# dymensionxyz/cometbft

Measured on AMD Instinct MI355X. Metric: Ed25519 verifs/sec at 1/2/4/8 GPUs + p50 VerifyCommit latency, 150 vals, higher is better.
Workload: dtype u32

## Files before the change

### cometbft_amd/_native.py

```python
from __future__ import annotations

import ctypes
import os

_HERE = os.path.dirname(os.path.abspath(__file__))
LIB_PATH = os.environ.get("CMTV_LIBRARY") or os.path.join(_HERE, "libcmtverify.so")

CMTV_OK = 0
CMTV_EINVAL = -1
CMTV_ENODEV = -2
CMTV_ENOMEM = -3
CMTV_EHIP = -4
CMTV_ERCCL = -5
CMTV_ECOMMIT = -6

MODE_GO_STDLIB = 0
MODE_ZIP215 = 1

VERIFY_COMMIT = 0
VERIFY_COMMIT_LIGHT = 1
VERIFY_COMMIT_LIGHT_TRUSTING = 2

KEY_ED25519 = 0
KEY_SECP256K1 = 1
# ... 39 lines not shown
                ("flags", ctypes.c_uint32), ("reserved", ctypes.c_uint32)]


class cmtv_stats(ctypes.Structure):
    _fields_ = [("calls", ctypes.c_uint64), ("signatures", ctypes.c_uint64), ("invalid", ctypes.c_uint64),
                ("kernel_launches", ctypes.c_uint64), ("device_ms", ctypes.c_double),
                ("last_kernel_ms", ctypes.c_double), ("cache_hits", ctypes.c_uint64),
                ("cache_entries", ctypes.c_uint64), ("keyed_launches", ctypes.c_uint64),
                ("sharded_calls", ctypes.c_uint64), ("gathers", ctypes.c_uint64),
                ("faults_injected", ctypes.c_uint64), ("n_devices", ctypes.c_uint32), ("rccl", ctypes.c_uint32),
                ("fused_sign_bytes", ctypes.c_uint64), ("device_failures", ctypes.c_uint64),
                ("reshards", ctypes.c_uint64), ("late_k_waves", ctypes.c_uint64),
                ("live_devices", ctypes.c_uint32), ("secp_batch_launches", ctypes.c_uint32),
                ("timed_calls", ctypes.c_uint64), ("rccl_failures", ctypes.c_uint64),
                ("polled_calls", ctypes.c_uint64), ("direct_chunks", ctypes.c_uint64),
                ("masked_chunks", ctypes.c_uint64), ("isolated_calls", ctypes.c_uint64)]


class cmtv_device_stats(ctypes.Structure):
    _fields_ = [("ordinal", ctypes.c_int32), ("failed", ctypes.c_uint32), ("calls", ctypes.c_uint64),
                ("signatures", ctypes.c_uint64), ("kernel_launches", ctypes.c_uint64),
                ("device_ms", ctypes.c_double), ("timed_calls", ctypes.c_uint64)]


_u8p = ctypes.POINTER(ctypes.c_uint8)


class cmtv_block_id(ctypes.Structure):
    _fields_ = [("hash", _u8p), ("hash_len", ctypes.c_uint32), ("psh_total", ctypes.c_uint32),
                ("psh_hash", _u8p), ("psh_hash_len", ctypes.c_uint32)]

# ... 151 lines not shown
```

### cometbft_amd/csrc/hs_helper.h

```cpp
#pragma once
#include "devtables.h"
#include "quad.h"

namespace cmtv {

constexpr int kHsCombPre = 6, kHsCombPreFused = 3, kHsCombPreSr = 0;
constexpr uint32_t kHsSlotU2 = 3 * 5 * 64;
constexpr uint32_t kHsTabU2 = 2 * 9 * 5 * 64;

__device__ __forceinline__ int hs_comb_pre(uint32_t hs_tune, int dflt) {
  const int c = (hs_tune & 0xFFu) ? (int)(hs_tune & 0xFFu) - 1 : dflt;
  return c > 16 ? 16 : c;
}

__device__ __forceinline__ int hs_workgroup_windows(uint32_t flags, uint32_t t) {
  const bool wide = __ballot(t < 48 && (flags & 2u) != 0) != 0;
  int W = HS_WINDOWS;
#pragma unroll 1
  for (int x = HS_WINDOWS; x < HS_MAX_WINDOWS; x++) W += __ballot(t < 48 && (int)((flags >> 8) & 0xFFu) > x) ? 1 : 0;
  return wide ? HS_WIDE_WINDOWS : W;
}

template <class Clock>
__device__ __forceinline__ void hs_helper_windows(const SigPrep& p, int W, const BComb16& bc, const uint2* tabs,
                                                  uint2* ring, uint32_t t, const Clock& clock, uint64_t& hwait) {
  const uint32_t slot = t < 48 ? t : 47;
  const bool r_flip = (p.flags & 1u) != 0;
  uint32_t tA[8], tR[8];
  hs_digits16(tA, p.k1, W);
  hs_digits16(tR, p.k2, W);
  sc_shift_out(tA, 4);
  sc_shift_out(tR, 4);
  const uint2* tw = tabs + (slot >> 4) * kHsTabU2;
  const uint32_t qb = 4 * (slot & 15);
  auto rd = [&](int P, int e, int c, fe& r) {
    const uint2* src = tw + (P * 9 + e) * 5 * 64 + qb + c;
#pragma unroll
    for (int k = 0; k < 5; k++) {
      const uint2 x = src[k * 64];
      r.v[2 * k] = x.x;
      r.v[2 * k + 1] = x.y;
    }
  };
  auto put = [&](uint2* dst, const fe* out) {
    if (t < 48) {
#pragma unroll
      for (int c = 0; c < 4; c++)
#pragma unroll
        for (int k = 0; k < 5; k++)
          dst[(slot >> 4) * 320 + k * 64 + qb + c] = make_uint2(out[c].v[2 * k], out[c].v[2 * k + 1]);
    }
  };
#pragma unroll 1
  for (int win = W - 2; win >= 0; win--) {
    const int dA = (int)sc_shift_out(tA, 4) - 8;
    const int dR = (int)sc_shift_out(tR, 4) - 8;
    fe out[4];
    h_window_addend(out, rd, dA, dR, r_flip);
    put(ring + (win & 1) * kHsSlotU2, out);
    const uint64_t c0 = clock();
    __syncthreads();
    hwait += clock() - c0;
  }
  fe out[4], d2;
  fe_sub(out[0], bc.P.Y, bc.P.X);
  fe_add(out[1], bc.P.Y, bc.P.X);
  fe_add(out[2], bc.P.Z, bc.P.Z);
  fe_const_d2(d2);
  fe_mul(out[3], bc.P.T, d2);
  put(ring + kHsSlotU2, out);
}

__device__ __forceinline__ void hs_slot_load(const uint2* sl, uint32_t wave, uint32_t t, fe& c) {
#pragma unroll
  for (int k = 0; k < 5; k++) {
    const uint2 x = sl[wave * 320 + k * 64 + t];
    c.v[2 * k] = x.x;
    c.v[2 * k + 1] = x.y;
  }
}

}
```

### cometbft_amd/csrc/kernels.h

```cpp
#pragma once
#include <hip/hip_runtime.h>
#include <stdint.h>

namespace cmtv {

constexpr uint32_t kBtabWords = (3 * 128 + 3 * 32768 + 16 * 32768) * 36;
constexpr uint32_t kAtabWordsPerLane = 320;
constexpr uint32_t kCombWords = 32 * 128 * 32;
constexpr uint32_t kCombScratchWordsPerKey = 128 * 320;

constexpr uint32_t kFormLane = 0, kFormQuad = 1, kFormOct2 = 2, kFormRow = 3, kFormRow4 = 4;
constexpr uint32_t kFormMask = 0xFF, kLaunchForceWide = 0x100;
constexpr uint32_t kKeyedRow = 0, kKeyedQuad = 1, kKeyedLane = 2;

constexpr uint32_t kRowSlots = 256, kRowSlotWords = 1024, kRowMaxCap = 4 * (kRowSlotWords - 16);
struct RowSlot {
  uint32_t* words = nullptr;
  uint64_t* tagged = nullptr;
  uint32_t seq = 0;
};

struct SbFuse {
  const void* tmpls = nullptr;
  const uint8_t* blob = nullptr;
  const uint32_t* tidx = nullptr;
  const uint8_t* flag = nullptr;
  const int64_t* sec = nullptr;
  const int32_t* nanos = nullptr;
};
constexpr uint32_t kSbFuseMaxMsg = 192;

constexpr uint32_t kDiagLateK = 0, kDiagWords = 4;
constexpr uint32_t kKeyedWaitDefault = 1u << 22;

hipError_t launch_btab_init(uint32_t* d_rows, hipStream_t s);
hipError_t launch_verify(uint32_t mode, uint32_t n, const void* pk, const void* sig, const void* msg,
                         const void* off, const uint32_t* btab, uint32_t* atab, void* valid, void* bitmap,
                         uint32_t kflags, hipStream_t s, const SbFuse* sb = nullptr, const RowSlot* row_slot = nullptr);
hipError_t launch_comb_build(uint32_t n_keys, const void* keys_pk, uint8_t* keys_ok, uint32_t* tabs,
                             uint32_t* scratch, bool negate, hipStream_t s);
hipError_t launch_verify_keyed(uint32_t mode, uint32_t n, uint32_t n_keys, const void* key_idx, const void* sig,
                               const void* msg, const void* off, const uint32_t* keys_pk, const uint8_t* keys_ok,
                               const uint32_t* ktabs, void* valid, void* bitmap, uint32_t form, uint32_t k_wait,
                               uint32_t* diag, uint32_t batch_kb, uint32_t* scr, const uint32_t* wtabs,
                               const uint32_t* btab, hipStream_t s, const RowSlot* row_slot = nullptr,
                               const SbFuse* sb = nullptr);
hipError_t launch_verify_keyed_lane(uint32_t mode, uint32_t n, uint32_t n_keys, const uint32_t* ki,
                                    const uint32_t* sgp, const uint8_t* mp, const uint32_t* op,
                                    const uint32_t* keys_pk, const uint8_t* keys_ok, const uint32_t* ktabs,
                                    uint8_t* vp, uint64_t* bp, uint32_t batch_kb, uint32_t* scr,
                                    const uint32_t* wtabs, const uint32_t* btab, hipStream_t s);
constexpr size_t kWideTableWords = (size_t)16 * 32768 * 32;
constexpr size_t kWideScratchWordsPerKey = (size_t)16 * (32768 / 64) * 64 * 10;
// ... 41 lines not shown
```

### cometbft_amd/csrc/kernels.hip

```cpp
#include <hip/hip_runtime.h>

#include "devtables.h"
#include "hs_helper.h"
#include "kernel_parts.h"
#include "kernels.h"
#include "phase_probe.h"
#include "quad.h"
#include "signbytes.h"
#include "verify_core.h"

CMTV_PHASE_BUFFER()

#ifndef CMTV_QUAD_WAVES_PER_EU
#define CMTV_QUAD_WAVES_PER_EU 1
#endif

#ifndef CMTV_VERIFY_WAVES_PER_EU
#define CMTV_VERIFY_WAVES_PER_EU 2
#endif

namespace cmtv {

template <uint32_t MODE>
__global__ __launch_bounds__(64, CMTV_VERIFY_WAVES_PER_EU) void k_verify(uint32_t n, const uint32_t* __restrict__ pk,
// ... 81 lines not shown
        qwait += CMTV_CLOCK() - c0;
        hs_slot_load(xbuf + (win & 1) * kHsSlotU2, wave, t, c);
      },
      [&](fe& c) {
        CMTV_STAMP(3);
        __syncthreads();
        CMTV_STAMP(4);
        hs_slot_load(xbuf + kHsSlotU2, wave, t, c);
      });
  CMTV_STAMP(5);
  CMTV_STAMP_VAL(6, qwait);
  quad_verdict_store(v, active, s, n, wave, t, out_valid, out_bitmap, tags);
}

template <uint32_t MODE>
__global__ __launch_bounds__(128, CMTV_QUAD_WAVES_PER_EU) void k_verify_oct_split(
    uint32_t n, const uint32_t* __restrict__ pk, const uint32_t* __restrict__ sig, const uint8_t* __restrict__ msg,
    const uint32_t* __restrict__ off, const uint32_t* __restrict__ btab, uint8_t* __restrict__ out_valid,
    uint64_t* __restrict__ out_bitmap, uint32_t force_wide, SbFuse sb) {
  CMTV_URGENT();
  const uint32_t t = threadIdx.x & 63;
  const uint32_t gid = blockIdx.x * 64 + t;
  const uint32_t s = gid >> 3;
  const bool active = s < n;
  const uint32_t i = active ? s : n - 1;
  __shared__ uint32_t prep[8][SIG_PREP_WORDS + 1];
  __shared__ uint32_t bpt[8][40];
  __shared__ uint2 tab_lds[9 * 5 * 64];
  __shared__ uint32_t sbm[8][kSbFuseMaxMsg / 4];
  if (threadIdx.x >= 64) {
// ... 221 lines not shown
  CMTV_STAMP(3);
  __syncthreads();
  CMTV_STAMP(4);
  const uint32_t cb = bpt_limb(bpt, t);
  bool v_ok = r_join4<MODE>(x, v, xh[0][t], xh[1][t], cb, (p.flags & 4u) != 0 && a_ok && r_ok, r_canon);
  CMTV_STAMP(5);
  CMTV_STAMP_RT(6);
  const bool active = s < n;
  v_ok = v_ok && active;
  if (t == 0 && active && out_valid) out_valid[s] = v_ok ? 1 : 0;
  if (out_bitmap && active) row_bitmap_add(slot, s, n, v_ok, out_bitmap, t);
}

hipError_t launch_verify(uint32_t mode, uint32_t n, const void* pk, const void* sig, const void* msg,
                         const void* off, const uint32_t* btab, uint32_t* atab, void* valid, void* bitmap,
                         uint32_t kflags, hipStream_t s, const SbFuse* sb, const RowSlot* row_slot) {
  const SbFuse fz = sb ? *sb : SbFuse{};
  const uint32_t form = kflags & kFormMask;
  const uint32_t fw = (kflags & kLaunchForceWide) ? 1u : 0u;
  if (n == 0) return hipSuccess;
  auto pkp = static_cast<const uint32_t*>(pk);
  auto sgp = static_cast<const uint32_t*>(sig);
  auto mp = static_cast<const uint8_t*>(msg);
  auto op = static_cast<const uint32_t*>(off);
  auto vp = static_cast<uint8_t*>(valid);
  auto bp = static_cast<uint64_t*>(bitmap);
  const RowSlot rs = row_slot ? *row_slot : RowSlot{};
  if ((form == kFormRow4 || form == kFormRow) && (n > kRowMaxCap || (bp && !rs.words))) return hipErrorInvalidValue;
  if (form != kFormLane && form != kFormQuad && form != kFormOct2 && form != kFormRow && form != kFormRow4)
    return hipErrorInvalidValue;
  if (fz.tmpls && form == kFormLane) return hipErrorInvalidValue;
// ... 2 lines not shown
    switch (form) {
      case kFormRow4:
        hipLaunchKernelGGL(k_verify_row4_split<M>, dim3(n), dim3(256), 0, s, n, pkp, sgp, mp, op, btab, vp, bp, fw, fz,
                           rs);
        break;
      case kFormRow:
        hipLaunchKernelGGL(k_verify_row_split<M>, dim3((n + 2) / 3), dim3(256), 0, s, n, pkp, sgp, mp, op, btab, vp, bp,
                           fw, fz, rs);
        break;
      case kFormOct2:
        hipLaunchKernelGGL(k_verify_oct_split<M>, dim3(((n + 63) / 64) * 8), dim3(128), 0, s, n, pkp, sgp, mp, op, btab,
                           vp, bp, fw, fz);
        break;
      case kFormQuad: {
        const uint32_t slices = 4 * ((n + 63) / 64);
        hipLaunchKernelGGL(k_verify_quad_hs<M>, dim3((slices + 2) / 3), dim3(256), 0, s, n, pkp, sgp, mp, op, btab, vp,
                           bp, fw, fz, kflags >> 16, rs);
        break;
      }
      default:
        hipLaunchKernelGGL(k_verify<M>, dim3((n + 63) / 64), dim3(64), 0, s, n, pkp, sgp, mp, op, btab, atab, vp, bp);
    }
  });
  return hipGetLastError();
}

}
```

### cometbft_amd/csrc/launch.cpp

```cpp
#include "runtime_state.h"

namespace cmtv {

struct LaunchScope {
  cmtv_ctx* ctx;
  CmtvDev& D;
  hipStream_t s;
  Timing::Pair tp{};
  bool timed = false;
  hipError_t begin() {
    D.timing.harvest(ctx->stats, D.device_ms, D.timed_calls, false);
    timed = ctx->timing_every && D.timing_seq++ % ctx->timing_every == 0;
    return timed ? D.timing.begin(tp, s) : hipSuccess;
  }
  hipError_t launched(hipError_t e) {
    if (e != hipSuccess) {
      D.timing.abandon(tp);
      return e;
    }
    ctx->stats.kernel_launches++;
    D.launches++;
    return hipSuccess;
  }
  int finish(size_t n, Scratch* lane_scratch) {
// ... 50 lines not shown
  return e;
}

int enqueue_verify(cmtv_ctx* ctx, CmtvDev& D, size_t n, const uint8_t* d_pk, const uint8_t* d_sig,
                   const uint8_t* d_msg, const uint32_t* d_off, uint32_t mode, uint8_t* d_valid, uint64_t* d_bitmap,
                   hipStream_t s, const SbFuse* sb, Scratch* scr) {
  Scratch& S = scr ? *scr : D.scratch;
  if (n == 0) return CMTV_OK;
  if (fault_hit(ctx) || D.inject_fault) return CMTV_EHIP;
  if (sb && (mode == kModeSr25519 || !fuse_ok(ctx, n))) return CMTV_EINVAL;
  const bool sr = mode == kModeSr25519;
  const uint32_t form = sr ? sr_form(ctx, n) : ed_form(ctx, n);
  const bool lane = form == kFormLane;
  const bool row = form == kFormRow || form == kFormRow4;
  const uint32_t kflags = form | (form == kFormQuad ? ctx->hs_tune << 16 : 0u) |
                          (ctx->force_wide ? kLaunchForceWide : 0u);
  hipError_t e = hipSuccess;
  if (lane) {
    const size_t lanes = std::min<size_t>(n, ctx->lane_chunk);
    const size_t lanes_padded = (lanes + 63) / 64 * 64;
    if ((e = acquire_scratch(S, lanes_padded * kAtabWordsPerLane * sizeof(uint32_t), s)) != hipSuccess)
      return hip_fail(e);
  }
  RowSlot slot;
  uint32_t slot_k = 0;
  if (row && (e = row_slot_acquire(ctx, D, s, d_bitmap != nullptr, slot, slot_k)) != hipSuccess) return hip_fail(e);
  const bool qtag = ctx->quad_poll && !sr && form == kFormQuad && d_bitmap && D.tag_arm && n <= kChunk;
  if (qtag) {
    slot = RowSlot{};
    take_tags(D, slot, 16);
  }
  LaunchScope L{ctx, D, s};
  if ((e = L.begin()) != hipSuccess) return hip_fail(e);
  const size_t chunk = lane ? ctx->lane_chunk : kChunk;
  for (size_t c = 0; c < n; c += chunk) {
    const uint32_t cn = (uint32_t)std::min<size_t>(chunk, n - c);
    if (sr)
      e = launch_verify_sr25519(cn, d_pk + 32 * c, d_sig + 64 * c, d_msg, d_off + c, D.d_btab,
                                static_cast<uint32_t*>(S.buf.p), D.d_srprog, ctx->sr_nops,
                                d_valid ? d_valid + c : nullptr, d_bitmap ? d_bitmap + c / 64 : nullptr, kflags, s);
    else
      e = launch_verify(mode, cn, d_pk + 32 * c, d_sig + 64 * c, d_msg, d_off + c, D.d_btab,
                        static_cast<uint32_t*>(S.buf.p), d_valid ? d_valid + c : nullptr,
                        d_bitmap ? d_bitmap + c / 64 : nullptr, kflags, s, sb, row || qtag ? &slot : nullptr);
    if (e == hipSuccess && row) e = row_slot_release(ctx, D, s, slot_k);
    if ((e = L.launched(e)) != hipSuccess) return hip_fail(e);
  }
  return L.finish(n, lane ? &S : nullptr);
}

int enqueue_verify_keyed(cmtv_ctx* ctx, CmtvDev& D, const cmtv_keyset::PerDev& K, size_t n_keys, size_t n,
                         const uint32_t* d_idx, const uint8_t* d_sig, const uint8_t* d_msg, const uint32_t* d_off,
                         uint32_t mode, uint8_t* d_valid, uint64_t* d_bitmap, hipStream_t s, Scratch* scr,
                         const SbFuse* sb, uint32_t min_waves) {
  if (n == 0) return CMTV_OK;
  if (!min_waves) min_waves = ctx->keyed_batch_min_waves;
  Scratch& S = scr ? *scr : D.scratch;
  if (sb && !keyed_fuse_ok(ctx, n)) return CMTV_EINVAL;
  if (!d_idx && !sb) return CMTV_EINVAL;
// ... 158 lines not shown
```

### cometbft_amd/csrc/phase_probe.h

```cpp
#pragma once

#ifdef CMTV_PHASE_PROBE
#define CMTV_PHASE_BUFFER(suffix)                                                                          \
  namespace cmtv {                                                                                         \
  constexpr int kPhaseSlots = 8;                                                                           \
  static __device__ uint64_t g_phase[4096 * 4 * kPhaseSlots];                                              \
  }                                                                                                        \
  extern "C" int cmtv_debug_phase_times##suffix(uint64_t* out, size_t n) {                                 \
    const size_t cap = sizeof(cmtv::g_phase) / sizeof(uint64_t);                                           \
    if (n > cap) n = cap;                                                                                  \
    if (hipDeviceSynchronize() != hipSuccess) return -1;                                                   \
    return hipMemcpyFromSymbol(out, HIP_SYMBOL(cmtv::g_phase), n * sizeof(uint64_t), 0,                    \
                               hipMemcpyDeviceToHost) == hipSuccess                                        \
               ? 0                                                                                         \
               : -1;                                                                                       \
  }
#define CMTV_PHASE_PUT(waves, cap, k, val)                                                                 \
  do {                                                                                                     \
    if ((threadIdx.x & 63) == 0 && blockIdx.x < (cap))                                                     \
      g_phase[((size_t)blockIdx.x * (waves) + (threadIdx.x >> 6)) * kPhaseSlots + (k)] = (val);            \
  } while (0)
#define CMTV_CLOCK() __builtin_amdgcn_s_memtime()
#define CMTV_STAMP(k) CMTV_PHASE_PUT(4, 4096, k, CMTV_CLOCK())
#define CMTV_STAMP_RT(k) CMTV_PHASE_PUT(4, 4096, k, __builtin_amdgcn_s_memrealtime())
#define CMTV_STAMP_VAL(k, val) CMTV_PHASE_PUT(4, 4096, k, val)
#define CMTV_STAMP5(k) CMTV_PHASE_PUT(5, 3200, k, CMTV_CLOCK())
#define CMTV_HWID5()                                                                                       \
  do {                                                                                                     \
    uint32_t hwid_;                                                                                        \
    asm volatile("s_getreg_b32 %0, hwreg(HW_REG_HW_ID)" : "=s"(hwid_));                                     \
    CMTV_PHASE_PUT(5, 3200, 6, hwid_);                                                                     \
  } while (0)
#else
#define CMTV_PHASE_BUFFER(suffix)
#define CMTV_STAMP(k) ((void)0)
#define CMTV_STAMP_RT(k) ((void)0)
#define CMTV_STAMP_VAL(k, val) ((void)0)
#define CMTV_STAMP5(k) ((void)0)
#define CMTV_HWID5() ((void)0)
#define CMTV_CLOCK() 0ull
#endif
```

### cometbft_amd/csrc/quad.h

```cpp
#pragma once
#include "halfscalar.h"
#include "verify_core.h"

namespace cmtv {

constexpr int QP_B0 = 0x00, QP_B1 = 0x55, QP_B2 = 0xAA, QP_B3 = 0xFF;
constexpr int QP_SWAP01 = (1 << 0) | (0 << 2) | (2 << 4) | (3 << 6);

constexpr int qp(int s0, int s1, int s2, int s3) { return s0 | (s1 << 2) | (s2 << 4) | (s3 << 6); }

CMTV_HD uint32_t fe_p2(int i) { return i == 0 ? P2_0 : ((i & 1) ? P2_O : P2_E); }

CMTV_HD void fe_pick(fe& h, int lane, const fe& a, const fe& b, const fe& c, const fe& d) {
  const bool l1 = lane & 1, l2 = lane & 2;
#pragma unroll
  for (int i = 0; i < 10; i++) {
    const uint32_t lo = l1 ? b.v[i] : a.v[i];
    const uint32_t hi = l1 ? d.v[i] : c.v[i];
    h.v[i] = l2 ? hi : lo;
  }
}

CMTV_HD void q_identity(fe& v, int lane) {
  fe_0(v);
// ... 272 lines not shown
    d[j] = p.k1[j];
    d[8 + j] = p.k2[j];
    d[16 + j] = p.u[j];
  }
  d[24] = p.flags;
}
CMTV_HD void sig_prep_load(SigPrep& p, const uint32_t* d) {
#pragma unroll
  for (int j = 0; j < 8; j++) {
    p.k1[j] = d[j];
    p.k2[j] = d[8 + j];
    p.u[j] = d[16 + j];
  }
  p.flags = d[24];
}

template <class BTab>
CMTV_HD void q_bcomb16(ge_p3& P, const uint32_t u[8], const BTab& btab) {
  uint32_t lo[8], hi[8];
  hs_digits65536(lo, hi, u);
  p3_identity(P);
  ge_efgh t;
#pragma unroll 1
  for (int j = 15; j >= 0; j--) {
    const int d = (int)(j >= 8 ? sc_shift_out(hi, 16) : sc_shift_out(lo, 16)) - 0x8000;
    const int ib = d < 0 ? -d : d;
    ge_add_table<false>(t, P, btab, BC16_BASE + j * BT16_ENTRIES + (ib > 0 ? ib - 1 : 0), d < 0, ib == 0);
    efgh_to_p3(P, t);
  }
}
// ... 3 lines not shown
  uint32_t lo[8], hi[8];
  int j;
  CMTV_HD void init(const uint32_t u[8]) {
    hs_digits65536(lo, hi, u);
    p3_identity(P);
    j = 15;
  }
  template <class BTab>
  CMTV_HD void step(const BTab& btab) {
    const int d = (int)(j >= 8 ? sc_shift_out(hi, 16) : sc_shift_out(lo, 16)) - 0x8000;
    const int ib = d < 0 ? -d : d;
    ge_efgh t;
    ge_add_table<false>(t, P, btab, BC16_BASE + j * BT16_ENTRIES + (ib > 0 ? ib - 1 : 0), d < 0, ib == 0);
    efgh_to_p3(P, t);
    j--;
  }
};

CMTV_HD void bpoint_store(uint32_t* d, const ge_p3& P) {
  fe c[4], d2;
  fe_sub(c[0], P.Y, P.X);
  fe_add(c[1], P.Y, P.X);
  fe_add(c[2], P.Z, P.Z);
  fe_const_d2(d2);
  fe_mul(c[3], P.T, d2);
#pragma unroll
  for (int k = 0; k < 3; k++) fe_carry(c[k]);
#pragma unroll
  for (int k = 0; k < 4; k++)
#pragma unroll
// ... 293 lines not shown
      b_ident = ib == 0;
    }
#pragma unroll 1
    for (int d = 0; d < 4; d++) q_dbl(q, v);
    get_s(win, c);
    q_add(q, v, c);
    if (has_b) {
      q_niels_fix(cB, lane, b_neg, b_ident);
      q_add(q, v, cB);
    }
  }
  get_b(c);
  q_add(q, v, c);
}

template <uint32_t MODE, class Q, class BTab, class ATab, class GetPrep, class GetS, class GetB>
CMTV_HD bool q_verify_hs(const Q& q, const uint32_t* pk_ptr, const uint32_t* sig_ptr, const BTab& btab, ATab& tabA,
                         ATab& tabR, int j0, const GetPrep& get_prep, const GetS& get_s, const GetB& get_b) {
  const int lane = q.lane();
  uint32_t w[8];
  const uint32_t* src = (lane & 1) ? sig_ptr : pk_ptr;
#pragma unroll
  for (int i = 0; i < 8; i++) w[i] = src[i];
  fe v, rc;
  bool a_ok, r_ok, r_canon;
  {
    ge_p3 P;
    const bool dec = p3_frombytes(P, w);
    const bool canon = y_is_canonical(w) && !(fe_iszero(P.X) && (w[7] >> 31));
    fe x, y, t, one;
    fe_1(one);
    q.template perm<QP_B0>(x, P.X);
    q.template perm<QP_B0>(y, P.Y);
    q.template perm<QP_B0>(t, P.T);
    fe_pick(v, lane, x, y, one, t);
    q.template perm<QP_B1>(x, P.X);
    q.template perm<QP_B1>(y, P.Y);
    q.template perm<QP_B1>(t, P.T);
    fe_pick(rc, lane, x, y, one, t);
    a_ok = q.template perm32<QP_B0>(dec ? 1u : 0u) != 0;
    r_ok = q.template perm32<QP_B1>(dec ? 1u : 0u) != 0;
    r_canon = q.template perm32<QP_B1>(canon ? 1u : 0u) != 0;
    const bool xt = lane == 0 || lane == 3;
    fe_neg(t, v);
    fe_carry(t);
    fe_select(v, v, t, xt);
    fe_neg(t, rc);
    fe_carry(t);
    fe_select(rc, rc, t, xt);
  }
  SigPrep p;
  q_hs_straus(q, v, rc, btab, tabA, tabR, j0, p, get_prep, get_s, get_b);
  const bool s_ok = (p.flags & 4u) != 0;
  if (MODE == MODE_ZIP215) {
    const bool so = q_small_order(q, v);
    return s_ok && a_ok && r_ok && so;
  }
  fe z;
  q.template perm<QP_B2>(z, v);
  const bool x0 = fe_iszero(v);
  const bool yz = fe_equal(v, z);
  const bool e0 = q.template perm32<QP_B0>(x0 ? 1u : 0u) != 0;
  const bool e1 = q.template perm32<QP_B1>(yz ? 1u : 0u) != 0;
  return s_ok && a_ok && r_ok && r_canon && e0 && e1;
}

template <uint32_t MODE, class Q, class BTab, class ATab, class Probe = NullProbe>
CMTV_HD bool q_verify(const Q& q, const uint32_t* pk_ptr, const uint32_t* sig_ptr, const uint8_t* msg,
                      uint32_t mlen, const BTab& btab, ATab& tabA, ATab& tabR, const Probe& probe = Probe(),
                      bool force_wide = false) {
  return q_verify_split<MODE>(
      q, pk_ptr, sig_ptr, btab, tabA, tabR,
      [&](SigPrep& p) { q_prepare<MODE>(p, pk_ptr, sig_ptr, msg, mlen, force_wide); }, NoExtB(), probe);
}

}
```

### cometbft_amd/csrc/runtime.cpp

```cpp
#include <climits>
#include <cstdio>
#include <cstdlib>
#include <new>
#include <thread>

#include "runtime_state.h"
#include "merlin.h"

namespace cmtv {

uint64_t phase_now(const cmtv_ctx* ctx) { return phase_clock(ctx); }

void phase_add(cmtv_ctx* ctx, int phase, uint64_t t0) {
  if (!ctx->phases_on || !t0) return;
  ctx->phase_ns[phase] += phase_clock(ctx) - t0;
  if (phase == kPhPrepare) ctx->phase_calls++;
}

void phase_add_ns(cmtv_ctx* ctx, int phase, uint64_t ns) {
  if (!ctx->phases_on) return;
  ctx->phase_ns[phase] += ns;
  if (phase == kPhPipePlan) ctx->phase_calls++;
}

// ... 172 lines not shown
    if (end != hp && *end == 0 && v >= 0 && v <= 16) ctx->hs_tune = (uint32_t)(v + 1);
  }
  if (const char* lc = std::getenv("CMTV_LANE_CHUNK")) {
    const size_t v = (size_t)std::strtoull(lc, nullptr, 10) / 64 * 64;
    if (v >= 64 && v <= kChunk) ctx->lane_chunk = v;
  }
  if (const char* sm = std::getenv("CMTV_SHARD_MIN")) ctx->shard_min = (size_t)std::strtoull(sm, nullptr, 10);
  if (const char* fa = std::getenv("CMTV_FAULT_AT")) ctx->fault_at = (uint64_t)std::strtoull(fa, nullptr, 10);
  env_is("CMTV_FORCE_WIDE", '1', ctx->force_wide);
  env_not("CMTV_NO_SB_FUSE", '1', ctx->sb_fuse);
  env_not("CMTV_NO_ZC_IN", '1', ctx->zc_in);
  env_not("CMTV_ZC_HOST_IN", '0', ctx->zc_host_in);
  env_not("CMTV_EARLY_SIGS", '0', ctx->early_sigs);
  if (const char* hp = std::getenv("CMTV_HOST_POLL")) ctx->host_poll = std::atoi(hp) != 0;
  if (const char* kl = std::getenv("CMTV_FORCE_K_LATE")) ctx->keyed_wait = kl[0] == '1' ? 0u : kKeyedWaitDefault;
  env_int("CMTV_KEYED_BATCH_MIN_WAVES", 1, 1l << 20, ctx->keyed_batch_min_waves);
  env_int("CMTV_KEYED_BATCH_MIN_WAVES", 1, 1l << 20, ctx->secp_batch_min_waves);
  if (std::getenv("CMTV_KEYED_BATCH_MIN_WAVES")) ctx->secp_batch_max_kb = 8;
  env_not("CMTV_ROW_FENCE", '0', ctx->row_fence);
  env_is("CMTV_HOST_PHASES", '1', ctx->phases_on);
  if (const char* tm = std::getenv("CMTV_TIMING")) {
    const long v = std::strtol(tm, nullptr, 10);
    ctx->timing_every = v < 0 ? 0u : (uint32_t)std::min<long>(v, 1l << 20);
  }
  if (const char* fs = std::getenv("CMTV_FAULT_SYNC_DEV")) {
    char* end = nullptr;
    const long g = std::strtol(fs, &end, 10);
    if (end != fs && g >= 0) ctx->fault_sync_dev = g;
  }
  ctx->force_rccl = std::getenv("CMTV_FORCE_RCCL") != nullptr;
// ... 234 lines not shown
int cmtv_sync(cmtv_ctx* ctx) {
  if (!ctx) return CMTV_EINVAL;
  std::lock_guard<std::mutex> g(ctx->mu);
  for (auto& D : ctx->devs) {
    if (D.failed) continue;
    if (hipSetDevice(D.ordinal) != hipSuccess) return CMTV_ENODEV;
    const hipError_t e = hipStreamSynchronize(D.stream);
    if (e != hipSuccess) return hip_fail(e);
  }
  harvest(ctx, false);
  (void)hipSetDevice(ctx->devs[0].ordinal);
  return CMTV_OK;
}

static void read_diag(cmtv_ctx* ctx) {
  uint64_t late = 0;
  for (auto& D : ctx->devs) {
    if (D.failed || !D.d_diag) continue;
    (void)hipSetDevice(D.ordinal);
    uint32_t w[kDiagWords] = {};
    if (hipMemcpy(w, D.d_diag, sizeof(w), hipMemcpyDeviceToHost) == hipSuccess) late += w[kDiagLateK];
  }
  ctx->stats.late_k_waves = late;
}

int cmtv_stats_get(cmtv_ctx* ctx, cmtv_stats* out) {
  if (!ctx || !out) return CMTV_EINVAL;
  std::lock_guard<std::mutex> g(ctx->mu);
  harvest(ctx, true);
  read_diag(ctx);
  (void)hipSetDevice(ctx->devs[0].ordinal);
  ctx->stats.cache_entries = ctx->cache.size();
  ctx->stats.live_devices = (uint32_t)ctx->live.size();
  *out = ctx->stats;
  return CMTV_OK;
}

int cmtv_device_stats_get(cmtv_ctx* ctx, int g, cmtv_device_stats* out) {
// ... 236 lines not shown
```

### cometbft_amd/csrc/runtime_state.h

```cpp
#pragma once
#include <hip/hip_runtime.h>

#include <algorithm>
#include <array>
#include <atomic>
#include <chrono>
#include <cstring>
#include <deque>
#include <map>
#include <memory>
#include <mutex>
#include <random>
#include <string>
#include <unordered_map>
#include <vector>

#include "../../include/cmtverify.h"
#include "host_pool.h"
#include "kernels.h"
#include "runtime_internal.h"

namespace cmtv {

constexpr uint32_t kChunk = 1u << 18;
// ... 248 lines not shown
  double device_ms = 0;
  uint64_t timing_seq = 0;
  BulkLane bulk;
};

}

struct cmtv_ctx {
  std::vector<cmtv::CmtvDev> devs;
  bool rccl = false;
  uint32_t default_mode = CMTV_MODE_GO_STDLIB;
  std::mutex mu;
  cmtv_stats stats{};
  uint32_t force_form = cmtv::kNoForm, force_keyed = cmtv::kNoForm;
  uint32_t hs_tune = 0;
  size_t lane_chunk = cmtv::kChunk;
  size_t shard_min = cmtv::kShardMinDefault;
  int sr_nops = 0;
  cmtv::VerdictCache cache;
  size_t keyset_cap = 0;
  std::vector<std::pair<std::string, cmtv_keyset*>> keysets;
  std::vector<cmtv_secp_keyset*> secp_keysets;
  uint64_t fault_at = 0, launch_seq = 0;
  bool fault_pending = false;
  bool force_rccl = false, no_rccl = false, no_rccl_fallback = false;
  std::string rccl_lib;
  bool rccl_broken = false;
  uint32_t rccl_drain_ms = 2000;
  bool force_wide = false;
  bool sb_fuse = true;
// ... 181 lines not shown
```

### include/cmtverify.h

```cpp
#ifndef CMTVERIFY_H
#define CMTVERIFY_H

#include <stddef.h>
#include <stdint.h>

#ifdef __cplusplus
extern "C" {
#endif

#define CMTV_ABI_VERSION 11

enum {
  CMTV_OK = 0,
  CMTV_EINVAL = -1,
  CMTV_ENODEV = -2,
  CMTV_ENOMEM = -3,
  CMTV_EHIP = -4,
  CMTV_ERCCL = -5,
  CMTV_ECOMMIT = -6
};

enum { CMTV_MODE_GO_STDLIB = 0, CMTV_MODE_ZIP215 = 1 };

typedef struct cmtv_ctx cmtv_ctx;
// ... 22 lines not shown
  uint64_t faults_injected;
  uint32_t n_devices;
  uint32_t rccl;
  uint64_t fused_sign_bytes;
  uint64_t device_failures;
  uint64_t reshards;
  uint64_t late_k_waves;
  uint32_t live_devices;
  uint32_t secp_batch_launches;
  uint64_t timed_calls;
  uint64_t rccl_failures;
  uint64_t polled_calls;
  uint64_t direct_chunks;
  uint64_t masked_chunks;
  uint64_t isolated_calls;
} cmtv_stats;

typedef struct cmtv_device_stats {
  int32_t ordinal;
  uint32_t failed;
  uint64_t calls;
  uint64_t signatures;
  uint64_t kernel_launches;
  double device_ms;
  uint64_t timed_calls;
} cmtv_device_stats;


int cmtv_open(const cmtv_config* cfg, cmtv_ctx** out);

// ... 187 lines not shown
```

Baseline: 46.54 million.

## Add fifth wave that precomputes fixed-base [s]B comb prefix in quad HS kernel

Adds a k_verify_quad_hs_fold kernel with 320 threads, enabled by default through hs_fold. The extra fifth wave computes the first comb_pre rows of the fixed-base s·B comb per signature and publishes the partial point to LDS behind a workgroup flag. The verify waves do the remaining comb rows themselves, then spin-wait on the flag and fold in the precomputed partial. If the flag is late they fall back to computing those rows locally and bump a diag counter. The intent is to take fixed-base work off the critical path of the quad waves, at the cost of a fifth wave per block, more LDS use, and a polling wait.

New measurement: 48.24 million (median of 6 runs). 1.04x the previous value.

```diff
diff --git a/cometbft_amd/_native.py b/cometbft_amd/_native.py
--- a/cometbft_amd/_native.py
+++ b/cometbft_amd/_native.py
@@ -77,7 +77,8 @@
                 ("live_devices", ctypes.c_uint32), ("secp_batch_launches", ctypes.c_uint32),
                 ("timed_calls", ctypes.c_uint64), ("rccl_failures", ctypes.c_uint64),
                 ("polled_calls", ctypes.c_uint64), ("direct_chunks", ctypes.c_uint64),
-                ("masked_chunks", ctypes.c_uint64), ("isolated_calls", ctypes.c_uint64)]
+                ("masked_chunks", ctypes.c_uint64), ("isolated_calls", ctypes.c_uint64),
+                ("late_ps_waves", ctypes.c_uint64)]
 
 
 class cmtv_device_stats(ctypes.Structure):
diff --git a/cometbft_amd/csrc/hs_helper.h b/cometbft_amd/csrc/hs_helper.h
--- a/cometbft_amd/csrc/hs_helper.h
+++ b/cometbft_amd/csrc/hs_helper.h
@@ -7,6 +7,9 @@
 constexpr int kHsCombPre = 6, kHsCombPreFused = 3, kHsCombPreSr = 0;
 constexpr uint32_t kHsSlotU2 = 3 * 5 * 64;
 constexpr uint32_t kHsTabU2 = 2 * 9 * 5 * 64;
+
+constexpr uint32_t kHsPsWords = 30;
+constexpr int kHsFoldCombPre = 16;
 
 __device__ __forceinline__ int hs_comb_pre(uint32_t hs_tune, int dflt) {
   const int c = (hs_tune & 0xFFu) ? (int)(hs_tune & 0xFFu) - 1 : dflt;
@@ -21,9 +24,19 @@
   return wide ? HS_WIDE_WINDOWS : W;
 }
 
+__device__ __forceinline__ void hs_slot_store(uint2* dst, uint32_t t, const fe* out) {
+  if (t < 48) {
+#pragma unroll
+    for (int c = 0; c < 4; c++)
+#pragma unroll
+      for (int k = 0; k < 5; k++)
+        dst[(t >> 4) * 320 + k * 64 + 4 * (t & 15) + c] = make_uint2(out[c].v[2 * k], out[c].v[2 * k + 1]);
+  }
+}
+
 template <class Clock>
-__device__ __forceinline__ void hs_helper_windows(const SigPrep& p, int W, const BComb16& bc, const uint2* tabs,
-                                                  uint2* ring, uint32_t t, const Clock& clock, uint64_t& hwait) {
+__device__ __forceinline__ void hs_helper_sums(const SigPrep& p, int W, const uint2* tabs, uint2* ring, uint32_t t,
+                                               const Clock& clock, uint64_t& hwait) {
   const uint32_t slot = t < 48 ? t : 47;
   const bool r_flip = (p.flags & 1u) != 0;
   uint32_t tA[8], tR[8];
@@ -42,33 +55,30 @@
       r.v[2 * k + 1] = x.y;
     }
   };
-  auto put = [&](uint2* dst, const fe* out) {
-    if (t < 48) {
-#pragma unroll
-      for (int c = 0; c < 4; c++)
-#pragma unroll
-        for (int k = 0; k < 5; k++)
-          dst[(slot >> 4) * 320 + k * 64 + qb + c] = make_uint2(out[c].v[2 * k], out[c].v[2 * k + 1]);
-    }
-  };
 #pragma unroll 1
   for (int win = W - 2; win >= 0; win--) {
     const int dA = (int)sc_shift_out(tA, 4) - 8;
     const int dR = (int)sc_shift_out(tR, 4) - 8;
     fe out[4];
     h_window_addend(out, rd, dA, dR, r_flip);
-    put(ring + (win & 1) * kHsSlotU2, out);
+    hs_slot_store(ring + (win & 1) * kHsSlotU2, t, out);
     const uint64_t c0 = clock();
     __syncthreads();
     hwait += clock() - c0;
   }
+}
+
+template <class Clock>
+__device__ __forceinline__ void hs_helper_windows(const SigPrep& p, int W, const BComb16& bc, const uint2* tabs,
+                                                  uint2* ring, uint32_t t, const Clock& clock, uint64_t& hwait) {
+  hs_helper_sums(p, W, tabs, ring, t, clock, hwait);
   fe out[4], d2;
   fe_sub(out[0], bc.P.Y, bc.P.X);
   fe_add(out[1], bc.P.Y, bc.P.X);
   fe_add(out[2], bc.P.Z, bc.P.Z);
   fe_const_d2(d2);
   fe_mul(out[3], bc.P.T, d2);
-  put(ring + kHsSlotU2, out);
+  hs_slot_store(ring + kHsSlotU2, t, out);
 }
 
 __device__ __forceinline__ void hs_slot_load(const uint2* sl, uint32_t wave, uint32_t t, fe& c) {
diff --git a/cometbft_amd/csrc/kernels.h b/cometbft_amd/csrc/kernels.h
--- a/cometbft_amd/csrc/kernels.h
+++ b/cometbft_amd/csrc/kernels.h
@@ -10,7 +10,7 @@
 constexpr uint32_t kCombScratchWordsPerKey = 128 * 320;
 
 constexpr uint32_t kFormLane = 0, kFormQuad = 1, kFormOct2 = 2, kFormRow = 3, kFormRow4 = 4;
-constexpr uint32_t kFormMask = 0xFF, kLaunchForceWide = 0x100;
+constexpr uint32_t kFormMask = 0xFF, kLaunchForceWide = 0x100, kLaunchHsFold = 0x200;
 constexpr uint32_t kKeyedRow = 0, kKeyedQuad = 1, kKeyedLane = 2;
 
 constexpr uint32_t kRowSlots = 256, kRowSlotWords = 1024, kRowMaxCap = 4 * (kRowSlotWords - 16);
@@ -30,13 +30,14 @@
 };
 constexpr uint32_t kSbFuseMaxMsg = 192;
 
-constexpr uint32_t kDiagLateK = 0, kDiagWords = 4;
-constexpr uint32_t kKeyedWaitDefault = 1u << 22;
+constexpr uint32_t kDiagLateK = 0, kDiagLatePs = 1, kDiagWords = 4;
+constexpr uint32_t kKeyedWaitDefault = 1u << 22, kPsWaitDefault = 1u << 22;
 
 hipError_t launch_btab_init(uint32_t* d_rows, hipStream_t s);
 hipError_t launch_verify(uint32_t mode, uint32_t n, const void* pk, const void* sig, const void* msg,
                          const void* off, const uint32_t* btab, uint32_t* atab, void* valid, void* bitmap,
-                         uint32_t kflags, hipStream_t s, const SbFuse* sb = nullptr, const RowSlot* row_slot = nullptr);
+                         uint32_t kflags, hipStream_t s, const SbFuse* sb = nullptr, const RowSlot* row_slot = nullptr,
+                         uint32_t ps_wait = kPsWaitDefault, uint32_t* diag = nullptr);
 hipError_t launch_comb_build(uint32_t n_keys, const void* keys_pk, uint8_t* keys_ok, uint32_t* tabs,
                              uint32_t* scratch, bool negate, hipStream_t s);
 hipError_t launch_verify_keyed(uint32_t mode, uint32_t n, uint32_t n_keys, const void* key_idx, const void* sig,
diff --git a/cometbft_amd/csrc/kernels.hip b/cometbft_amd/csrc/kernels.hip
--- a/cometbft_amd/csrc/kernels.hip
+++ b/cometbft_amd/csrc/kernels.hip
@@ -119,6 +119,138 @@
 }
 
 template <uint32_t MODE>
+__global__ __launch_bounds__(320, 1) void k_verify_quad_hs_fold(
+    uint32_t n, const uint32_t* __restrict__ pk, const uint32_t* __restrict__ sig, const uint8_t* __restrict__ msg,
+    const uint32_t* __restrict__ off, const uint32_t* __restrict__ btab, uint8_t* __restrict__ out_valid,
+    uint64_t* __restrict__ out_bitmap, uint32_t force_wide, SbFuse sb, uint32_t hs_tune, uint32_t ps_wait,
+    uint32_t* __restrict__ diag, RowSlot tags) {
+  CMTV_URGENT();
+  const uint32_t hw = threadIdx.x >> 6, t = threadIdx.x & 63;
+  const uint32_t base = blockIdx.x * 48;
+  const uint32_t tune = hs_tune >> 8;
+  const int comb_pre = hs_comb_pre(hs_tune, kHsFoldCombPre);
+  const uint32_t helper_wave = (tune & 1u) ? 3u : 0u;
+  __shared__ uint32_t prep[48][SIG_PREP_WORDS + 1];
+  __shared__ uint2 tab_lds[3][kHsTabU2];
+  __shared__ uint2 xbuf[2 * kHsSlotU2];
+  __shared__ uint32_t ps_ready;
+  static_assert(sizeof(xbuf) >= 48 * (kSbFuseMaxMsg + 4 * kHsPsWords), "P_s goes behind the sign-bytes buffer");
+  uint32_t* pspt = reinterpret_cast<uint32_t*>(xbuf) + 48 * (kSbFuseMaxMsg / 4);
+  CMTV_STAMP5(0);
+  CMTV_HWID5();
+  if (threadIdx.x == 0) ps_ready = 0u;
+  __syncthreads();
+  if (hw == 4) {
+    if (tune & 2u) __builtin_amdgcn_s_setprio(0);
+    if (tune & 4u) __builtin_amdgcn_s_setprio(3);
+    if (ps_wait != 0) {
+      const uint32_t slot = t < 48 ? t : 47;
+      const uint32_t s = base + slot;
+      const uint32_t i = s < n ? s : n - 1;
+      uint32_t sw[8];
+      load_words(sw, sig + 16 * (size_t)i + 8, 2);
+      const DevBTab bt{btab};
+      BComb16Ahead bc;
+      bc.init(sw, bt);
+#pragma unroll 1
+      for (int k = 0; k < comb_pre; k++) bc.step(bt);
+      if (t < 48) {
+#pragma unroll
+        for (int j = 0; j < 10; j++) {
+          pspt[t * kHsPsWords + j] = bc.P.X.v[j];
+          pspt[t * kHsPsWords + 10 + j] = bc.P.Y.v[j];
+          pspt[t * kHsPsWords + 20 + j] = bc.P.Z.v[j];
+        }
+      }
+      __builtin_amdgcn_fence(__ATOMIC_RELEASE, "workgroup");
+      if (t == 0) __hip_atomic_store(&ps_ready, 1u, __ATOMIC_RELAXED, __HIP_MEMORY_SCOPE_WORKGROUP);
+    }
+    CMTV_STAMP5(3);
+    CMTV_STAMP5(1);
+    __syncthreads();
+    CMTV_STAMP5(2);
+    const int W = (int)__builtin_amdgcn_readfirstlane((prep[0][24] >> 16) & 0xFFu);
+#pragma unroll 1
+    for (int win = W - 2; win >= 0; win--) __syncthreads();
+    return;
+  }
+  if (hw == helper_wave) {
+    const uint32_t slot = t < 48 ? t : 47;
+    const uint32_t s = base + slot;
+    const uint32_t i = s < n ? s : n - 1;
+    const uint8_t* mp;
+    uint32_t ml;
+    helper_message(sb, i, msg, off, reinterpret_cast<uint32_t*>(xbuf) + slot * (kSbFuseMaxMsg / 4), mp, ml);
+    SigPrep p;
+    q_prepare<MODE>(p, pk + 8 * (size_t)i, sig + 16 * (size_t)i, mp, ml, force_wide != 0);
+    const int W = hs_workgroup_windows(p.flags, t);
+    p.flags |= (uint32_t)W << 16;
+    if (t < 48) sig_prep_store_pair(prep[t], p);
+    CMTV_STAMP5(1);
+    __syncthreads();
+    CMTV_STAMP5(2);
+    uint64_t hwait = 0;
+    hs_helper_sums(p, W, &tab_lds[0][0], xbuf, t, [] { return (uint64_t)CMTV_CLOCK(); }, hwait);
+    CMTV_STAMP5_VAL(7, hwait);
+    CMTV_STAMP5(3);
+    return;
+  }
+  const uint32_t wave = hw - (hw > helper_wave ? 1u : 0u);
+  const uint32_t ls = wave * 16 + (t >> 2);
+  const uint32_t s = base + ls;
+  const bool active = s < n;
+  const uint32_t i = active ? s : n - 1;
+  DevQuad q;
+  DevATabQ ta{tab_lds[wave], t}, tr{tab_lds[wave] + 9 * 5 * 64, t};
+  uint64_t qwait = 0;
+  (void)qwait;
+  bool v = q_verify_hs_fold<MODE>(
+      q, pk + 8 * (size_t)i, sig + 16 * (size_t)i, DevBTabQ{btab}, 16 - comb_pre, ta, tr,
+      [&](fe& ps) {
+        const uint64_t c0 = CMTV_CLOCK();
+        (void)c0;
+        bool ready = false;
+        for (uint32_t spins = 0; spins < ps_wait; spins++) {
+          ready = __hip_atomic_load(&ps_ready, __ATOMIC_RELAXED, __HIP_MEMORY_SCOPE_WORKGROUP) != 0u;
+          if (ready) break;
+          __builtin_amdgcn_s_sleep(2);
+        }
+        CMTV_STAMP5_VAL(3, CMTV_CLOCK() - c0);
+        if (__builtin_expect(__ballot(ready) != __ballot(1), 0)) {
+          if (t == 0 && diag) atomicAdd(diag + kDiagLatePs, 1u);
+          return false;
+        }
+        __builtin_amdgcn_fence(__ATOMIC_ACQUIRE, "workgroup");
+        const int lane = (int)(t & 3);
+        const uint32_t* pp = pspt + ls * kHsPsWords;
+        fe a, b;
+#pragma unroll
+        for (int j = 0; j < 10; j++) {
+          a.v[j] = pp[10 * q_p2_factor_a(lane) + j];
+          b.v[j] = pp[10 * q_p2_factor_b(lane) + j];
+        }
+        fe_mul(ps, a, b);
+        CMTV_STAMP5(4);
+        return true;
+      },
+      [&](SigPrep& p) {
+        CMTV_STAMP5(1);
+        __syncthreads();
+        CMTV_STAMP5(2);
+        sig_prep_load_pair(p, prep[ls]);
+      },
+      [&](int win, fe& c) {
+        const uint64_t c0 = CMTV_CLOCK();
+        __syncthreads();
+        qwait += CMTV_CLOCK() - c0;
+        hs_slot_load(xbuf + (win & 1) * kHsSlotU2, wave, t, c);
+      });
+  CMTV_STAMP5(5);
+  CMTV_STAMP5_VAL(7, qwait);
+  quad_verdict_store(v, active, s, n, wave, t, out_valid, out_bitmap, tags);
+}
+
+template <uint32_t MODE>
 __global__ __launch_bounds__(128, CMTV_QUAD_WAVES_PER_EU) void k_verify_oct_split(
     uint32_t n, const uint32_t* __restrict__ pk, const uint32_t* __restrict__ sig, const uint8_t* __restrict__ msg,
     const uint32_t* __restrict__ off, const uint32_t* __restrict__ btab, uint8_t* __restrict__ out_valid,
@@ -370,7 +502,8 @@
 
 hipError_t launch_verify(uint32_t mode, uint32_t n, const void* pk, const void* sig, const void* msg,
                          const void* off, const uint32_t* btab, uint32_t* atab, void* valid, void* bitmap,
-                         uint32_t kflags, hipStream_t s, const SbFuse* sb, const RowSlot* row_slot) {
+                         uint32_t kflags, hipStream_t s, const SbFuse* sb, const RowSlot* row_slot, uint32_t ps_wait,
+                         uint32_t* diag) {
   const SbFuse fz = sb ? *sb : SbFuse{};
   const uint32_t form = kflags & kFormMask;
   const uint32_t fw = (kflags & kLaunchForceWide) ? 1u : 0u;
@@ -403,8 +536,12 @@
         break;
       case kFormQuad: {
         const uint32_t slices = 4 * ((n + 63) / 64);
-        hipLaunchKernelGGL(k_verify_quad_hs<M>, dim3((slices + 2) / 3), dim3(256), 0, s, n, pkp, sgp, mp, op, btab, vp,
-                           bp, fw, fz, kflags >> 16, rs);
+        if (kflags & kLaunchHsFold)
+          hipLaunchKernelGGL(k_verify_quad_hs_fold<M>, dim3((slices + 2) / 3), dim3(320), 0, s, n, pkp, sgp, mp, op,
+                             btab, vp, bp, fw, fz, kflags >> 16, ps_wait, diag, rs);
+        else
+          hipLaunchKernelGGL(k_verify_quad_hs<M>, dim3((slices + 2) / 3), dim3(256), 0, s, n, pkp, sgp, mp, op, btab,
+                             vp, bp, fw, fz, kflags >> 16, rs);
         break;
       }
       default:
diff --git a/cometbft_amd/csrc/launch.cpp b/cometbft_amd/csrc/launch.cpp
--- a/cometbft_amd/csrc/launch.cpp
+++ b/cometbft_amd/csrc/launch.cpp
@@ -88,7 +88,7 @@
   const bool lane = form == kFormLane;
   const bool row = form == kFormRow || form == kFormRow4;
   const uint32_t kflags = form | (form == kFormQuad ? ctx->hs_tune << 16 : 0u) |
-                          (ctx->force_wide ? kLaunchForceWide : 0u);
+                          (ctx->force_wide ? kLaunchForceWide : 0u) | (ctx->hs_fold ? kLaunchHsFold : 0u);
   hipError_t e = hipSuccess;
   if (lane) {
     const size_t lanes = std::min<size_t>(n, ctx->lane_chunk);
@@ -116,7 +116,8 @@
     else
       e = launch_verify(mode, cn, d_pk + 32 * c, d_sig + 64 * c, d_msg, d_off + c, D.d_btab,
                         static_cast<uint32_t*>(S.buf.p), d_valid ? d_valid + c : nullptr,
-                        d_bitmap ? d_bitmap + c / 64 : nullptr, kflags, s, sb, row || qtag ? &slot : nullptr);
+                        d_bitmap ? d_bitmap + c / 64 : nullptr, kflags, s, sb, row || qtag ? &slot : nullptr,
+                        ctx->ps_wait, D.d_diag);
     if (e == hipSuccess && row) e = row_slot_release(ctx, D, s, slot_k);
     if ((e = L.launched(e)) != hipSuccess) return hip_fail(e);
   }
diff --git a/cometbft_amd/csrc/phase_probe.h b/cometbft_amd/csrc/phase_probe.h
--- a/cometbft_amd/csrc/phase_probe.h
+++ b/cometbft_amd/csrc/phase_probe.h
@@ -25,6 +25,7 @@
 #define CMTV_STAMP_RT(k) CMTV_PHASE_PUT(4, 4096, k, __builtin_amdgcn_s_memrealtime())
 #define CMTV_STAMP_VAL(k, val) CMTV_PHASE_PUT(4, 4096, k, val)
 #define CMTV_STAMP5(k) CMTV_PHASE_PUT(5, 3200, k, CMTV_CLOCK())
+#define CMTV_STAMP5_VAL(k, val) CMTV_PHASE_PUT(5, 3200, k, val)
 #define CMTV_HWID5()                                                                                       \
   do {                                                                                                     \
     uint32_t hwid_;                                                                                        \
@@ -37,6 +38,7 @@
 #define CMTV_STAMP_RT(k) ((void)0)
 #define CMTV_STAMP_VAL(k, val) ((void)0)
 #define CMTV_STAMP5(k) ((void)0)
+#define CMTV_STAMP5_VAL(k, val) ((void)0)
 #define CMTV_HWID5() ((void)0)
 #define CMTV_CLOCK() 0ull
 #endif
diff --git a/cometbft_amd/csrc/quad.h b/cometbft_amd/csrc/quad.h
--- a/cometbft_amd/csrc/quad.h
+++ b/cometbft_amd/csrc/quad.h
@@ -310,6 +310,23 @@
   }
   p.flags = d[24];
 }
+CMTV_HD void sig_prep_store_pair(uint32_t* d, const SigPrep& p) {
+#pragma unroll
+  for (int j = 0; j < 8; j++) {
+    d[j] = p.k1[j];
+    d[8 + j] = p.k2[j];
+  }
+  d[24] = p.flags;
+}
+CMTV_HD void sig_prep_load_pair(SigPrep& p, const uint32_t* d) {
+#pragma unroll
+  for (int j = 0; j < 8; j++) {
+    p.k1[j] = d[j];
+    p.k2[j] = d[8 + j];
+    p.u[j] = 0;
+  }
+  p.flags = d[24];
+}
 
 template <class BTab>
 CMTV_HD void q_bcomb16(ge_p3& P, const uint32_t u[8], const BTab& btab) {
@@ -343,6 +360,45 @@
     ge_add_table<false>(t, P, btab, BC16_BASE + j * BT16_ENTRIES + (ib > 0 ? ib - 1 : 0), d < 0, ib == 0);
     efgh_to_p3(P, t);
     j--;
+  }
+};
+
+struct BComb16Ahead {
+  struct Row {
+    fe c[3];
+    CMTV_HD void load_fe(int, int k, fe& r) const { fe_select(r, c[0], c[1], k == 1); fe_select(r, r, c[2], k == 2); }
+  };
+  ge_p3 P;
+  uint32_t lo[8], hi[8];
+  int j;
+  Row next;
+  bool neg, ident;
+  template <class BTab>
+  CMTV_HD void fetch(const BTab& btab) {
+    const int d = (int)(j >= 8 ? sc_shift_out(hi, 16) : sc_shift_out(lo, 16)) - 0x8000;
+    const int ib = d < 0 ? -d : d;
+    const int e = BC16_BASE + j * BT16_ENTRIES + (ib > 0 ? ib - 1 : 0);
+    neg = d < 0;
+    ident = ib == 0;
+#pragma unroll
+    for (int k = 0; k < 3; k++) btab.load_fe(e, k, next.c[k]);
+  }
+  template <class BTab>
+  CMTV_HD void init(const uint32_t u[8], const BTab& btab) {
+    hs_digits65536(lo, hi, u);
+    p3_identity(P);
+    j = 15;
+    fetch(btab);
+  }
+  template <class BTab>
+  CMTV_HD void step(const BTab& btab) {
+    const Row cur = next;
+    const bool c_neg = neg, c_ident = ident;
+    j--;
+    if (j >= 0) fetch(btab);
+    ge_efgh t;
+    ge_add_table<false>(t, P, cur, 0, c_neg, c_ident);
+    efgh_to_p3(P, t);
   }
 };
 
@@ -666,44 +722,41 @@
   q_add(q, v, c);
 }
 
-template <uint32_t MODE, class Q, class BTab, class ATab, class GetPrep, class GetS, class GetB>
-CMTV_HD bool q_verify_hs(const Q& q, const uint32_t* pk_ptr, const uint32_t* sig_ptr, const BTab& btab, ATab& tabA,
-                         ATab& tabR, int j0, const GetPrep& get_prep, const GetS& get_s, const GetB& get_b) {
+template <class Q>
+CMTV_HD void q_hs_decode(const Q& q, const uint32_t* pk_ptr, const uint32_t* sig_ptr, fe& v, fe& rc, bool& a_ok,
+                         bool& r_ok, bool& r_canon) {
   const int lane = q.lane();
   uint32_t w[8];
   const uint32_t* src = (lane & 1) ? sig_ptr : pk_ptr;
 #pragma unroll
   for (int i = 0; i < 8; i++) w[i] = src[i];
-  fe v, rc;
-  bool a_ok, r_ok, r_canon;
-  {
-    ge_p3 P;
-    const bool dec = p3_frombytes(P, w);
-    const bool canon = y_is_canonical(w) && !(fe_iszero(P.X) && (w[7] >> 31));
-    fe x, y, t, one;
-    fe_1(one);
-    q.template perm<QP_B0>(x, P.X);
-    q.template perm<QP_B0>(y, P.Y);
-    q.template perm<QP_B0>(t, P.T);
-    fe_pick(v, lane, x, y, one, t);
-    q.template perm<QP_B1>(x, P.X);
-    q.template perm<QP_B1>(y, P.Y);
-    q.template perm<QP_B1>(t, P.T);
-    fe_pick(rc, lane, x, y, one, t);
-    a_ok = q.template perm32<QP_B0>(dec ? 1u : 0u) != 0;
-    r_ok = q.template perm32<QP_B1>(dec ? 1u : 0u) != 0;
-    r_canon = q.template perm32<QP_B1>(canon ? 1u : 0u) != 0;
-    const bool xt = lane == 0 || lane == 3;
-    fe_neg(t, v);
-    fe_carry(t);
-    fe_select(v, v, t, xt);
-    fe_neg(t, rc);
-    fe_carry(t);
-    fe_select(rc, rc, t, xt);
-  }
-  SigPrep p;
-  q_hs_straus(q, v, rc, btab, tabA, tabR, j0, p, get_prep, get_s, get_b);
-  const bool s_ok = (p.flags & 4u) != 0;
+  ge_p3 P;
+  const bool dec = p3_frombytes(P, w);
+  const bool canon = y_is_canonical(w) && !(fe_iszero(P.X) && (w[7] >> 31));
+  fe x, y, t, one;
+  fe_1(one);
+  q.template perm<QP_B0>(x, P.X);
+  q.template perm<QP_B0>(y, P.Y);
+  q.template perm<QP_B0>(t, P.T);
+  fe_pick(v, lane, x, y, one, t);
+  q.template perm<QP_B1>(x, P.X);
+  q.template perm<QP_B1>(y, P.Y);
+  q.template perm<QP_B1>(t, P.T);
+  fe_pick(rc, lane, x, y, one, t);
+  a_ok = q.template perm32<QP_B0>(dec ? 1u : 0u) != 0;
+  r_ok = q.template perm32<QP_B1>(dec ? 1u : 0u) != 0;
+  r_canon = q.template perm32<QP_B1>(canon ? 1u : 0u) != 0;
+  const bool xt = lane == 0 || lane == 3;
+  fe_neg(t, v);
+  fe_carry(t);
+  fe_select(v, v, t, xt);
+  fe_neg(t, rc);
+  fe_carry(t);
+  fe_select(rc, rc, t, xt);
+}
+
+template <uint32_t MODE, class Q>
+CMTV_HD bool q_hs_final(const Q& q, const fe& v, bool s_ok, bool a_ok, bool r_ok, bool r_canon) {
   if (MODE == MODE_ZIP215) {
     const bool so = q_small_order(q, v);
     return s_ok && a_ok && r_ok && so;
@@ -717,6 +770,113 @@
   return s_ok && a_ok && r_ok && r_canon && e0 && e1;
 }
 
+template <uint32_t MODE, class Q, class BTab, class ATab, class GetPrep, class GetS, class GetB>
+CMTV_HD bool q_verify_hs(const Q& q, const uint32_t* pk_ptr, const uint32_t* sig_ptr, const BTab& btab, ATab& tabA,
+                         ATab& tabR, int j0, const GetPrep& get_prep, const GetS& get_s, const GetB& get_b) {
+  fe v, rc;
+  bool a_ok, r_ok, r_canon;
+  q_hs_decode(q, pk_ptr, sig_ptr, v, rc, a_ok, r_ok, r_canon);
+  SigPrep p;
+  q_hs_straus(q, v, rc, btab, tabA, tabR, j0, p, get_prep, get_s, get_b);
+  return q_hs_final<MODE>(q, v, (p.flags & 4u) != 0, a_ok, r_ok, r_canon);
+}
+
+
+CMTV_HD int q_p2_factor_a(int lane) { return lane == 3 ? 0 : lane; }
+CMTV_HD int q_p2_factor_b(int lane) { return lane == 3 ? 1 : 2; }
+
+template <class Q, class BTab>
+CMTV_HD void q_sbase16_add(const Q& q, fe& v, const uint32_t s[8], const BTab& btab, int j_hi, int j_lo) {
+  const int lane = q.lane();
+  uint32_t lo[8], hi[8];
+  hs_digits65536(lo, hi, s);
+#pragma unroll 1
+  for (int j = 15; j >= j_hi; j--) sc_shift_out(j >= 8 ? hi : lo, 16);
+  fe cn;
+  bool neg = false, ident = false;
+  auto fetch = [&](int j) {
+    const int d = (int)(j >= 8 ? sc_shift_out(hi, 16) : sc_shift_out(lo, 16)) - 0x8000;
+    const int ib = d < 0 ? -d : d;
+    const int row = BC16_BASE + j * BT16_ENTRIES + (ib > 0 ? ib - 1 : 0);
+    neg = d < 0;
+    ident = ib == 0;
+    q_niels_load(
+        q, cn, [&](int off, fe& r) { btab.load_coord(row, off, r); }, BTAB_COORD_WORDS, 2 * BTAB_COORD_WORDS, neg);
+  };
+  if (j_hi > j_lo) fetch(j_hi - 1);
+#pragma unroll 1
+  for (int j = j_hi - 1; j >= j_lo; j--) {
+    fe c = cn;
+    const bool c_neg = neg, c_ident = ident;
+    if (j > j_lo) fetch(j - 1);
+    q_niels_fix(c, lane, c_neg, c_ident);
+    q_add(q, v, c);
+  }
+}
+
+template <class Q, class BTab, class ATab, class GetPs, class GetPrep, class GetS>
+CMTV_HD void q_hs_straus_fold(const Q& q, fe& v, fe& rc, const uint32_t s[8], const BTab& btab, int j0, ATab& tabA,
+                              ATab& tabR, SigPrep& p, const GetPs& get_ps, const GetPrep& get_prep,
+                              const GetS& get_s) {
+  const int lane = q.lane();
+  q_build_table_p3(q, tabA, v);
+  q_sbase16_add(q, rc, s, btab, j0, 0);
+  fe c;
+  {
+    fe ps;
+    if (get_ps(ps)) {
+      q_to_cached(q, c, ps);
+      q_add(q, rc, c);
+    } else {
+      q_sbase16_add(q, rc, s, btab, 16, j0);
+    }
+  }
+  q_build_table_p3(q, tabR, rc);
+  get_prep(p);
+  const bool r_flip = (p.flags & 1u) != 0;
+  const int W = (p.flags >> 16) & 0xFFu ? (int)((p.flags >> 16) & 0xFFu) : q_wave_windows(q, p.flags);
+  uint32_t tA[8], tR[8];
+  hs_digits16(tA, p.k1, W);
+  hs_digits16(tR, p.k2, W);
+  {
+    const int dA = (int)sc_shift_out(tA, 4) - 8;
+    const int dR = (int)sc_shift_out(tR, 4) - 8;
+    tabA.load(dA < 0 ? -dA : dA, v);
+    fe t, r;
+    fe_neg(t, v);
+    fe_carry(t);
+    fe_select(v, v, t, dA < 0 && (lane == 0 || lane == 3));
+    tabR.load(dR < 0 ? -dR : dR, r);
+    fe_neg(t, r);
+    fe_carry(t);
+    fe_select(r, r, t, ((dR < 0) != r_flip) && (lane == 0 || lane == 3));
+    q_to_cached(q, c, r);
+    q_add(q, v, c);
+  }
+#pragma unroll 1
+  for (int win = W - 2; win >= 0; win--) {
+#pragma unroll 1
+    for (int d = 0; d < 4; d++) q_dbl(q, v);
+    get_s(win, c);
+    q_add(q, v, c);
+  }
+}
+
+template <uint32_t MODE, class Q, class BTab, class ATab, class GetPs, class GetPrep, class GetS>
+CMTV_HD bool q_verify_hs_fold(const Q& q, const uint32_t* pk_ptr, const uint32_t* sig_ptr, const BTab& btab, int j0,
+                              ATab& tabA, ATab& tabR, const GetPs& get_ps, const GetPrep& get_prep,
+                              const GetS& get_s) {
+  fe v, rc;
+  bool a_ok, r_ok, r_canon;
+  q_hs_decode(q, pk_ptr, sig_ptr, v, rc, a_ok, r_ok, r_canon);
+  uint32_t s[8];
+#pragma unroll
+  for (int i = 0; i < 8; i++) s[i] = sig_ptr[8 + i];
+  SigPrep p;
+  q_hs_straus_fold(q, v, rc, s, btab, j0, tabA, tabR, p, get_ps, get_prep, get_s);
+  return q_hs_final<MODE>(q, v, (p.flags & 4u) != 0, a_ok, r_ok, r_canon);
+}
+
 template <uint32_t MODE, class Q, class BTab, class ATab, class Probe = NullProbe>
 CMTV_HD bool q_verify(const Q& q, const uint32_t* pk_ptr, const uint32_t* sig_ptr, const uint8_t* msg,
                       uint32_t mlen, const BTab& btab, ATab& tabA, ATab& tabR, const Probe& probe = Probe(),
diff --git a/cometbft_amd/csrc/runtime.cpp b/cometbft_amd/csrc/runtime.cpp
--- a/cometbft_amd/csrc/runtime.cpp
+++ b/cometbft_amd/csrc/runtime.cpp
@@ -210,6 +210,13 @@
   env_not("CMTV_EARLY_SIGS", '0', ctx->early_sigs);
   if (const char* hp = std::getenv("CMTV_HOST_POLL")) ctx->host_poll = std::atoi(hp) != 0;
   if (const char* kl = std::getenv("CMTV_FORCE_K_LATE")) ctx->keyed_wait = kl[0] == '1' ? 0u : kKeyedWaitDefault;
+  env_not("CMTV_HS_FOLD", '0', ctx->hs_fold);
+  if (const char* pl = std::getenv("CMTV_FORCE_PS_LATE")) ctx->ps_wait = pl[0] == '1' ? 0u : kPsWaitDefault;
+  {
+    uint32_t ft = 0;
+    env_int("CMTV_HS_FOLD_TUNE", 0, 7, ft);
+    ctx->hs_tune |= ft << 8;
+  }
   env_int("CMTV_KEYED_BATCH_MIN_WAVES", 1, 1l << 20, ctx->keyed_batch_min_waves);
   env_int("CMTV_KEYED_BATCH_MIN_WAVES", 1, 1l << 20, ctx->secp_batch_min_waves);
   if (std::getenv("CMTV_KEYED_BATCH_MIN_WAVES")) ctx->secp_batch_max_kb = 8;
@@ -474,14 +481,18 @@
 }
 
 static void read_diag(cmtv_ctx* ctx) {
-  uint64_t late = 0;
+  uint64_t late = 0, late_ps = 0;
   for (auto& D : ctx->devs) {
     if (D.failed || !D.d_diag) continue;
     (void)hipSetDevice(D.ordinal);
     uint32_t w[kDiagWords] = {};
-    if (hipMemcpy(w, D.d_diag, sizeof(w), hipMemcpyDeviceToHost) == hipSuccess) late += w[kDiagLateK];
+    if (hipMemcpy(w, D.d_diag, sizeof(w), hipMemcpyDeviceToHost) == hipSuccess) {
+      late += w[kDiagLateK];
+      late_ps += w[kDiagLatePs];
+    }
   }
   ctx->stats.late_k_waves = late;
+  ctx->stats.late_ps_waves = late_ps;
 }
 
 int cmtv_stats_get(cmtv_ctx* ctx, cmtv_stats* out) {
diff --git a/cometbft_amd/csrc/runtime_state.h b/cometbft_amd/csrc/runtime_state.h
--- a/cometbft_amd/csrc/runtime_state.h
+++ b/cometbft_amd/csrc/runtime_state.h
@@ -286,6 +286,8 @@
   cmtv_stats stats{};
   uint32_t force_form = cmtv::kNoForm, force_keyed = cmtv::kNoForm;
   uint32_t hs_tune = 0;
+  bool hs_fold = true;
+  uint32_t ps_wait = cmtv::kPsWaitDefault;
   size_t lane_chunk = cmtv::kChunk;
   size_t shard_min = cmtv::kShardMinDefault;
   int sr_nops = 0;
diff --git a/include/cmtverify.h b/include/cmtverify.h
--- a/include/cmtverify.h
+++ b/include/cmtverify.h
@@ -60,6 +60,7 @@
   uint64_t direct_chunks;
   uint64_t masked_chunks;
   uint64_t isolated_calls;
+  uint64_t late_ps_waves;
 } cmtv_stats;
 
 typedef struct cmtv_device_stats {
```
